# NVIDIA/makani

Measured on AMD Instinct MI355X. Metric: SFNO train samples/sec at 721x1440x73ch, higher is better.
Workload: dtype bf16; 1 GPU; sfno_sc3_layers8_edim384; grid=721x1440, channels=73, global_batch=1, parallelism=dp1, spectral_arithmetic=x3, multistep_count=1, multistep_checkpoint=False, launch=hipGraph replay of the captured step, channel_gemm=hip (csrc/conv1x1.hip)

## Files before the change

include/makani_amd.h:

```cpp
#ifndef MAKANI_AMD_H
#define MAKANI_AMD_H

#ifdef __cplusplus
extern "C" {
#endif

#define MK_F32 0
#define MK_BF16 1

#define MK_EINVAL -1
#define MK_EUNSUP -2

#define MK_TRI_NONE 0
#define MK_TRI_ROW_GE 1
#define MK_TRI_K_GE 2
#define MK_TRI_ROW_LE 3
#define MK_TRI_K_LE 4

typedef struct MkGemm {
    const float* A;
    const float* B;
    float* C;
    long long a_batch, a_row, a_k;
    long long b_batch, b_col, b_k;
// ... 75 lines not shown
int mk_bias_gelu_fwd(const void* x, const float* bias, void* y, int dtype, long long planes, int channels,
                     long long hw, void* stream);
int mk_bias_gelu_bwd(const void* x, const float* bias, const void* gy, void* gx, float* sums, float* ws, int dtype,
                     long long planes, int channels, long long hw, void* stream);

int mk_quad_lp_chunks(long long hw);
int mk_quad_lp_fwd(const void* a, int a_dtype, const void* b, int b_dtype, const float* wgt, const float* q,
                   float* sums, float* ws, long long planes, long long hw, int mode, float p, void* stream);
int mk_quad_lp_bwd(const void* a, int a_dtype, const void* b, int b_dtype, const float* wgt, const float* q,
                   const float* g, void* da, void* db, long long planes, long long hw, int mode, float p, void* stream);

long long mk_spec_lp_blocks(int L, int M);
int mk_spec_lp_fwd(const float* S, const float* wgt, float* partial, int L, int M, long long R, int tri_off, int m_off,
                   float p, float w0, float w1, void* stream);
int mk_spec_lp_bwd(const float* S, const float* wgt, const float* g, float* dS, int L, int M, long long R, int tri_off,
                   int m_off, float p, float w0, float w1, void* stream);

int mk_spec_sep_mul(const float* x, const float* w, float* y, int L, int M, int Mw, int B, int Cp, int tri_off, int conj_w,
                    void* stream);
int mk_spec_sep_wgrad(const float* x, const float* gy, float* gw, int L, int M, int Mw, int B, int Cp, int tri_off, void* stream);
int mk_spec_diag_apply(const float* x, const float* w_c64, float* y, int L, int M, int B, int Cin, int Cout, int x_ld, int y_ld,
                       int y_pad, int tri_off, int dgrad, void* stream);
int mk_spec_diag_wgrad(const float* x, const float* gy, float* gw_c64, int L, int M, int B, int Cin, int Cout, int x_ld, int y_ld,
                       int tri_off, void* stream);

int mk_conv1x1_nn(const void* A, const void* X, void* Y, void* Ypre, const float* bias, const void* R, const void* G,
                  int M, int K, int lda, int B, long long N, int act, void* stream);
long long mk_conv1x1_wgrad_workspace(int M, int K, int B, long long N);
int mk_conv1x1_wgrad(const void* G, const void* X, float* dW, float* part, int M, int K, int B, long long N,
                     int accumulate, void* stream);
int mk_conv1x1_wgrad_fuses_bias(int M, int K, int B, long long N);
int mk_conv1x1_wgrad_bias(const void* G, const void* X, float* dW, float* dbias, float* part, int M, int K, int B, long long N,
                          int accumulate, void* stream);

int mk_adamw_step(float* p, const float* g, float* m, float* v, long long n, const float* grad_scale, float lr,
                  float beta1, float beta2, float eps, float weight_decay, int step, const float* step_state, void* stream);
int mk_adamw_advance(float* state, float beta1, float beta2, void* stream);
typedef struct MkAdamTensor {
    float* p;
    const float* g;
    float* m;
    float* v;
    long long n;
    void* p_bf16;
    void* p_bf16_t;
    int cols;
    int ld, ld_t;
} MkAdamTensor;
int mk_adamw_multi(const MkAdamTensor* tensors, int count, const float* grad_scale, float lr, float beta1, float beta2,
                   float eps, float weight_decay, int step, const float* step_state, void* stream);
long long mk_grad_norm_workspace(const MkAdamTensor* tensors, int count);
int mk_grad_clip_coef(const MkAdamTensor* tensors, int count, float max_norm, float* partial, float* out, void* stream);
long long mk_grad_norm_workspace_pre(const MkAdamTensor* tensors, int count, const MkAdamTensor* pre, int npre);
int mk_grad_clip_coef_pre(const MkAdamTensor* tensors, int count, const MkAdamTensor* pre, int npre, float max_norm, float* partial,
                          float* out, void* stream);

int mk_chan_layernorm_chunks(int C, long long P);
int mk_chan_layernorm_fwd(const void* x, int x_dtype, void* y, int y_dtype, float* stats, const float* gamma, const float* beta,
                          int B, int C, long long P, float eps, void* stream);
int mk_chan_layernorm_bwd(const void* x, int x_dtype, const void* gy, int g_dtype, void* gx, const float* stats,
                          const float* gamma, int B, int C, long long P, void* stream);
int mk_chan_layernorm_wgrad(const void* x, int x_dtype, const void* gy, int g_dtype, const float* stats, float* partial, int B,
                            int C, long long P, void* stream);

int mk_crps_chunks(long long hw);
int mk_crps(const void* f, int f_dtype, const void* obs, int o_dtype, const float* q, const float* w, const float* gout,
// ... 41 lines not shown
```

makani_amd/_lib.py:

```python
import ctypes as C
import os

import torch

_HERE = os.path.dirname(os.path.abspath(__file__))
LIB_PATH = os.environ.get("MAKANI_AMD_LIB") or os.path.join(_HERE, "libmakani_amd.so")

MK_F32, MK_BF16 = 0, 1
TRI_NONE, TRI_ROW_GE, TRI_K_GE, TRI_ROW_LE, TRI_K_LE = 0, 1, 2, 3, 4

c_ll, c_int, c_f, c_vp = C.c_longlong, C.c_int, C.c_float, C.c_void_p


class MkAdamTensor(C.Structure):
    _fields_ = [("p", C.c_void_p), ("g", C.c_void_p), ("m", C.c_void_p), ("v", C.c_void_p), ("n", C.c_longlong),
                ("p_bf16", C.c_void_p), ("p_bf16_t", C.c_void_p), ("cols", C.c_int), ("ld", C.c_int), ("ld_t", C.c_int)]


class MkGemm(C.Structure):
    _fields_ = [
        ("A", c_vp), ("B", c_vp), ("C", c_vp),
        ("a_batch", c_ll), ("a_row", c_ll), ("a_k", c_ll),
        ("b_batch", c_ll), ("b_col", c_ll), ("b_k", c_ll),
        ("c_batch", c_ll), ("c_row", c_ll), ("c_col", c_ll),
# ... 27 lines not shown
                      c_f, c_f, c_f, c_vp], c_int),
    "mk_irfft_rows": ([c_vp, c_vp, c_int, c_vp, C.POINTER(c_int), c_int, c_int, c_int, c_int, c_int, c_int, c_int,
                       c_f, c_f, c_f, c_vp], c_int),
    "mk_fft_seg_supported": ([c_int], c_int),
    "mk_rfft_rows_seg": ([c_vp, c_int, c_vp, c_vp, c_int, c_int, c_int, c_int, c_f, c_f, c_f, C.POINTER(MkFftSeg), c_vp], c_int),
    "mk_irfft_rows_seg": ([c_vp, c_vp, c_int, c_vp, c_int, c_int, c_int, c_int, c_f, c_f, c_f, C.POINTER(MkFftSeg), c_vp], c_int),
    "mk_weight_to_wlayout": ([c_vp, c_vp, c_int, c_int, c_int, c_int, c_int, c_vp], c_int),
    "mk_wlayout_to_weight_grad": ([c_vp, c_vp, c_int, c_int, c_int, c_int, c_int, c_vp], c_int),
    "mk_slayout_to_complex": ([c_vp, c_vp, c_int, c_int, c_int, c_int, c_int, c_int, c_int, c_vp], c_int),
    "mk_complex_to_slayout": ([c_vp, c_vp, c_int, c_int, c_int, c_int, c_int, c_vp], c_int),
    "mk_spec_sep_mul": ([c_vp, c_vp, c_vp, c_int, c_int, c_int, c_int, c_int, c_int, c_int, c_vp], c_int),
    "mk_spec_sep_wgrad": ([c_vp, c_vp, c_vp, c_int, c_int, c_int, c_int, c_int, c_int, c_vp], c_int),
    "mk_spec_diag_apply": ([c_vp, c_vp, c_vp, c_int, c_int, c_int, c_int, c_int, c_int, c_int, c_int, c_int, c_int, c_vp], c_int),
    "mk_spec_diag_wgrad": ([c_vp, c_vp, c_vp, c_int, c_int, c_int, c_int, c_int, c_int, c_int, c_int, c_vp], c_int),
    "mk_pointwise_chunks": ([c_ll, c_int, c_ll], c_int),
    "mk_plane_sums": ([c_vp, c_int, c_vp, c_vp, c_ll, c_ll, c_vp], c_int),
    "mk_instnorm_stats": ([c_vp, c_int, c_vp, c_vp, c_ll, c_ll, c_f, c_vp, c_f, c_vp], c_int),
    "mk_instnorm_merge": ([c_vp, c_vp, c_vp, c_ll, c_int, c_f, c_vp], c_int),
    "mk_instnorm_apply": ([c_vp, c_vp, c_int, c_vp, c_vp, c_vp, c_ll, c_int, c_ll, c_int, c_vp], c_int),
    "mk_instnorm_fused_chunks": ([c_ll, c_int, c_ll, c_int], c_int),
    "mk_instnorm_fwd_fused": ([c_vp, c_vp, c_int, c_vp, c_vp, c_vp, c_vp, c_vp, c_vp, c_ll, c_int, c_ll, c_f, c_int, c_vp], c_int),
    "mk_instnorm_bwd_fused": ([c_vp, c_vp, c_vp, c_int, c_vp, c_vp, c_vp, c_vp, c_vp, c_vp, c_vp, c_ll, c_int, c_ll, c_int, c_vp], c_int),
    "mk_instnorm_bwd": ([c_vp, c_vp, c_vp, c_int, c_vp, c_vp, c_vp, c_vp, c_vp, c_f, c_vp, c_vp, c_ll, c_int, c_ll, c_ll, c_int, c_int, c_vp], c_int),
    "mk_chan_layernorm_chunks": ([c_int, c_ll], c_int),
    "mk_chan_layernorm_fwd": ([c_vp, c_int, c_vp, c_int, c_vp, c_vp, c_vp, c_int, c_int, c_ll, c_f, c_vp], c_int),
    "mk_chan_layernorm_bwd": ([c_vp, c_int, c_vp, c_int, c_vp, c_vp, c_vp, c_int, c_int, c_ll, c_vp], c_int),
    "mk_chan_layernorm_wgrad": ([c_vp, c_int, c_vp, c_int, c_vp, c_vp, c_int, c_int, c_ll, c_vp], c_int),
    "mk_bias_gelu_fwd": ([c_vp, c_vp, c_vp, c_int, c_ll, c_int, c_ll, c_vp], c_int),
    "mk_conv1x1_nn": ([c_vp, c_vp, c_vp, c_vp, c_vp, c_vp, c_vp, c_int, c_int, c_int, c_int, c_ll, c_int, c_vp], c_int),
    "mk_conv1x1_wgrad_workspace": ([c_int, c_int, c_int, c_ll], c_ll),
    "mk_conv1x1_wgrad": ([c_vp, c_vp, c_vp, c_vp, c_int, c_int, c_int, c_ll, c_int, c_vp], c_int),
    "mk_conv1x1_wgrad_fuses_bias": ([c_int, c_int, c_int, c_ll], c_int),
    "mk_conv1x1_wgrad_bias": ([c_vp, c_vp, c_vp, c_vp, c_vp, c_int, c_int, c_int, c_ll, c_int, c_vp], c_int),
    "mk_adamw_step": ([c_vp, c_vp, c_vp, c_vp, c_ll, c_vp, c_f, c_f, c_f, c_f, c_f, c_int, c_vp, c_vp], c_int),
    "mk_adamw_advance": ([c_vp, c_f, c_f, c_vp], c_int),
    "mk_bias_gelu_bwd": ([c_vp, c_vp, c_vp, c_vp, c_vp, c_vp, c_int, c_ll, c_int, c_ll, c_vp], c_int),
    "mk_adamw_multi": ([c_vp, c_int, c_vp, c_f, c_f, c_f, c_f, c_f, c_int, c_vp, c_vp], c_int),
    "mk_instnorm_fwd": ([c_vp, c_vp, c_int, c_vp, c_vp, c_vp, c_vp, c_vp, c_vp, c_f, c_ll, c_int, c_ll, c_f, c_int, c_vp], c_int),
    "mk_grad_norm_workspace": ([c_vp, c_int], c_ll),
    "mk_grad_clip_coef": ([c_vp, c_int, c_f, c_vp, c_vp, c_vp], c_int),
    "mk_grad_norm_workspace_pre": ([c_vp, c_int, c_vp, c_int], c_ll),
    "mk_grad_clip_coef_pre": ([c_vp, c_int, c_vp, c_int, c_f, c_vp, c_vp, c_vp], c_int),
    "mk_spec_lp_blocks": ([c_int, c_int], c_ll),
    "mk_spec_lp_fwd": ([c_vp, c_vp, c_vp, c_int, c_int, c_ll, c_int, c_int, c_f, c_f, c_f, c_vp], c_int),
    "mk_spec_lp_bwd": ([c_vp, c_vp, c_vp, c_vp, c_int, c_int, c_ll, c_int, c_int, c_f, c_f, c_f, c_vp], c_int),
    "mk_crps_chunks": ([c_ll], c_int),
    "mk_crps": ([c_vp, c_int, c_vp, c_int, c_vp, c_vp, c_vp, c_vp, c_vp, c_int, c_int, c_int, c_ll, c_int, c_f, c_f, c_int, c_vp, c_vp], c_int),
    "mk_crps_complex": ([c_vp, c_vp, c_vp, c_vp, c_vp, c_vp, c_vp, c_int, c_int, c_int, c_ll, c_f, c_int, c_vp], c_int),
    "mk_disco_fwd": ([c_vp, c_vp, c_int, c_vp, c_vp, c_vp, c_vp, c_vp, c_vp, c_int, c_int, c_int, c_int, c_int, c_int, c_int, c_vp], c_int),
    "mk_disco_bwd": ([c_vp, c_vp, c_int, c_vp, c_vp, c_vp, c_vp, c_vp, c_int, c_int, c_int, c_int, c_int, c_int, c_vp], c_int),
    "mk_disco_bwd_same": ([c_vp, c_vp, c_int, c_vp, c_vp, c_vp, c_vp, c_vp, c_vp, c_int, c_int, c_int, c_int, c_int, c_int, c_vp], c_int),
    "mk_disco_runs_shape": ([c_int, c_int, c_int, c_int, c_int, c_vp, c_vp], c_int),
    "mk_disco_fused_shape": ([c_int, c_int, c_int, c_int, c_vp, c_vp], c_int),
    "mk_disco_fwd_fused": ([c_vp, c_vp, c_int, c_vp, c_vp, c_vp, c_vp, c_vp, c_int, c_int, c_int, c_int, c_int, c_int, c_vp], c_int),
    "mk_disco_fwd_runs": ([c_vp, c_vp, c_int, c_vp, c_vp, c_vp, c_vp, c_vp, c_int, c_int, c_int, c_int, c_int, c_int, c_int, c_int, c_int, c_vp], c_int),
    "mk_disco_bwd_runs": ([c_vp, c_vp, c_int, c_vp, c_vp, c_vp, c_vp, c_vp, c_int, c_int, c_int, c_int, c_int, c_int, c_int, c_int, c_int, c_int, c_vp], c_int),
    "mk_group_mix_supported": ([c_int, c_int], c_int),
    "mk_group_mix_blocks": ([c_ll, c_int, c_int], c_int),
    "mk_group_mix": ([c_vp, c_vp, c_vp, c_int, c_int, c_int, c_int, c_int, c_ll, c_vp], c_int),
    "mk_group_mix_wgrad": ([c_vp, c_vp, c_vp, c_int, c_int, c_int, c_int, c_int, c_ll, c_vp], c_int),
    "mk_resample_fwd": ([c_vp, c_vp, c_int, c_vp, c_vp, c_vp, c_vp, c_vp, c_vp, c_int, c_int, c_int, c_int, c_int, c_vp], c_int),
    "mk_resample_bwd": ([c_vp, c_vp, c_int, c_vp, c_vp, c_vp, c_vp, c_vp, c_vp, c_vp, c_vp, c_vp, c_int, c_int, c_int, c_int, c_int, c_vp], c_int),
    "mk_quad_lp_chunks": ([c_ll], c_int),
    "mk_quad_lp_fwd": ([c_vp, c_int, c_vp, c_int, c_vp, c_vp, c_vp, c_vp, c_ll, c_ll, c_int, c_f, c_vp], c_int),
    "mk_quad_lp_bwd": ([c_vp, c_int, c_vp, c_int, c_vp, c_vp, c_vp, c_vp, c_vp, c_ll, c_ll, c_int, c_f, c_vp], c_int),
}
# ... 74 lines not shown
```

makani_amd/csrc/conv1x1.hip:

```cpp
#include <stdlib.h>
#include <type_traits>

#include "common.h"

#ifndef MK_ASTAT_EPI_DRAIN
#define MK_ASTAT_EPI_DRAIN 0
#endif
#ifndef MK_A2_PRIO
#define MK_A2_PRIO 1
#endif
#ifndef MK_ASTAT_DIAG
#define MK_ASTAT_DIAG 0
#endif
#if MK_ASTAT_DIAG
__device__ unsigned long long g_astat_diag[16];
#define MK_AS_STAMP(k)                                              \
    do {                                                            \
        const unsigned long long t_ = __builtin_readcyclecounter(); \
        dg[k] += t_ - tprev;                                        \
        tprev = t_;                                                 \
    } while (0)
#else
#define MK_AS_STAMP(k)
#endif
// ... 1335 lines not shown
                store_tiles(ra[0], rb[0], 0);
                __syncthreads();
            }
        }
    }

    float* out = p.part + (long long)sp * p.M * p.K;
#pragma unroll
    for (int i = 0; i < 2; ++i)
#pragma unroll
        for (int j = 0; j < 2; ++j) {
            const int c = c0 + wn * 64 + j * 32 + l31;
#pragma unroll
            for (int r = 0; r < 16; ++r) {
                const int m = m0 + wm * 64 + i * 32 + (r & 3) + 8 * (r >> 2) + 4 * lh;
                if (m < p.M && c < p.K) out[(long long)m * p.K + c] = acc[i][j][r];
            }
        }
}

struct ConvWgR {
    const u16* P;
    const u16* Q;
    float* part;
    int RP, RQ, B, S, slabs, qslabs;
    int ldo;
    long long N;
    long long chunk;
    float* bias_part;
};


template <int WP, int WQ, int WTP, int WTQ, bool SWAP>
__global__ __launch_bounds__(512, 2) void conv_wgrad_ring_kernel(const ConvWgR p) {
#if defined(__HIP_DEVICE_COMPILE__)
    static_assert(WP * WQ == 8, "8 waves");
    constexpr int TP = WP * WTP * 32, TQ = WQ * WTQ * 32;
    constexpr int BK = 64;
    constexpr int STAGE = (TP + TQ) * 128;
    constexpr int NI = (TP + TQ) / 64;
    constexpr int NIP = TP / 64;
    static_assert(TP % 64 == 0 && TQ == 384, "row groups; Q is fetched by 2 x 3 DMA pieces per wave");
    __shared__ __attribute__((aligned(1024))) unsigned char smem[2 * STAGE];

    const int bid = xcd_remap(blockIdx.x, gridDim.x);
    const int slab = bid % p.slabs;
    const int qs = (bid / p.slabs) % p.qslabs;
    const int q0 = qs * TQ;
    const int sp = bid / (p.slabs * p.qslabs);
    const int splits_per_b = p.S / p.B;
    const int b = sp / splits_per_b;
    const long long nbeg = (long long)(sp % splits_per_b) * p.chunk;
    const long long nend = min(p.N, nbeg + p.chunk);
    const int nk = nbeg < nend ? (int)((nend - nbeg + BK - 1) / BK) : 0;

    const int tid = threadIdx.x, lane = tid & 63, wave = tid >> 6;
    const int wp = wave / WQ, wq = wave % WQ;
    const int l31 = lane & 31, lh = lane >> 5;

    const int c_log = (lane & 7) ^ ((((wave & 1) << 2) + (lane >> 4)) & 7);
    const unsigned rowbytes = (unsigned)(p.N * 2);
    unsigned voff[NI];
#pragma unroll
    for (int i = 0; i < NI; ++i) {
        const int rg = wave + 8 * i;
        int row;
        if (i < NIP) row = min(rg * 8 + (lane >> 3), p.RP - 1 - slab * TP);
        else row = min((rg - TP / 8) * 8 + (lane >> 3), p.RQ - 1 - q0);
        voff[i] = (unsigned)row * rowbytes + (unsigned)c_log * 16u;
    }
    const v4i_t rsP = make_rsrc(p.P + ((long long)b * p.RP + slab * TP) * p.N);
    const v4i_t rsQ = make_rsrc(p.Q + ((long long)b * p.RQ + q0) * p.N);
    const unsigned lds_w = lds_addr(smem) + __builtin_amdgcn_readfirstlane(wave) * 1024;

    auto issue = [&](int kt, int stage) {
        const long long n = nbeg + (long long)kt * BK;
        const unsigned soff = (unsigned)__builtin_amdgcn_readfirstlane((int)(unsigned)(n * 2));
        const unsigned dst = lds_w + stage * STAGE;
// ... 71 lines not shown
        asm volatile("s_waitcnt lgkmcnt(0)" ::: "memory");
        __builtin_amdgcn_s_barrier();
        if (kt + 2 < nk) issue(kt + 2, kt & 1);
    }

    if (bias_wave) {
        const int RG = SWAP ? p.RQ : p.RP;
#pragma unroll
        for (int i = 0; i < WTG; ++i) {
            const float tot = rsum[i] + __shfl_xor(rsum[i], 32);
            const int m = SWAP ? q0 + (wq * WTQ + i) * 32 + l31 : slab * TP + (wp * WTP + i) * 32 + l31;
            if (lh == 0 && m < RG) p.bias_part[((long long)sp * NSH + bshare) * RG + m] = tot;
        }
    }

    float* out = p.part + (long long)sp * ((long long)(SWAP ? p.RQ : p.RP) * p.ldo);
#pragma unroll
    for (int i = 0; i < WTP; ++i)
#pragma unroll
        for (int j = 0; j < WTQ; ++j) {
            const int prow0 = slab * TP + (wp * WTP + i) * 32, qrow0 = q0 + (wq * WTQ + j) * 32;
#pragma unroll
            for (int r = 0; r < 16; ++r) {
                const int rr = (r & 3) + 8 * (r >> 2) + 4 * lh;
                const int m = SWAP ? qrow0 + rr : prow0 + rr;
                const int k = SWAP ? prow0 + l31 : qrow0 + l31;
                const bool ok = SWAP ? (m < p.RQ && k < p.RP) : (m < p.RP && k < p.RQ);
                if (ok) out[(long long)m * p.ldo + k] = acc[i][j][r];
            }
        }
#endif
}

__global__ void reduce_splits(const float* __restrict__ part, float* __restrict__ out, long long n, int S, int accumulate) {
    const long long i = (long long)blockIdx.x * blockDim.x + threadIdx.x;
    if (i >= n) return;
    float s = accumulate ? out[i] : 0.f;
    int k = 0;
    for (; k + 8 <= S; k += 8) {
        float v[8];
#pragma unroll
        for (int u = 0; u < 8; ++u) v[u] = part[(long long)(k + u) * n + i];
#pragma unroll
        for (int u = 0; u < 8; ++u) s += v[u];
    }
    for (; k < S; ++k) s += part[(long long)k * n + i];
    out[i] = s;
}

__global__ void reduce_splits4(const float4* __restrict__ part, float4* __restrict__ out, long long n4, int S, int accumulate) {
    const long long i = (long long)blockIdx.x * blockDim.x + threadIdx.x;
    if (i >= n4) return;
    float4 s = accumulate ? out[i] : make_float4(0.f, 0.f, 0.f, 0.f);
    int k = 0;
    for (; k + 8 <= S; k += 8) {
        float4 v[8];
#pragma unroll
        for (int u = 0; u < 8; ++u) v[u] = part[(long long)(k + u) * n4 + i];
#pragma unroll
        for (int u = 0; u < 8; ++u) s.x += v[u].x, s.y += v[u].y, s.z += v[u].z, s.w += v[u].w;
    }
    for (; k < S; ++k) {
        const float4 v = part[(long long)k * n4 + i];
        s.x += v.x, s.y += v.y, s.z += v.z, s.w += v.w;
    }
    out[i] = s;
}

}

#if MK_ASTAT_DIAG
extern "C" int mk_astat_diag_read(unsigned long long* out, int reset) {
    if (hipMemcpyFromSymbol(out, HIP_SYMBOL(g_astat_diag), sizeof(unsigned long long) * 16) != hipSuccess) return 1;
    if (reset) {
        unsigned long long z[16] = {};
        if (hipMemcpyToSymbol(HIP_SYMBOL(g_astat_diag), z, sizeof(z)) != hipSuccess) return 1;
    }
    return 0;
}
#endif

extern "C" int mk_conv1x1_nn(const void* A, const void* X, void* Y, void* Ypre, const float* bias, const void* R,
                             const void* G, int M, int K, int lda, int B, long long N, int act, void* stream) {
    MK_REQUIRE(A && X && Y, "conv1x1_nn: null pointer");
    MK_REQUIRE(M > 0 && K > 0 && B > 0 && N > 0, "conv1x1_nn: bad shape M=%d K=%d B=%d N=%lld", M, K, B, N);
    MK_REQUIRE((lda % 8) == 0 && lda >= K, "conv1x1_nn: lda=%d must be a multiple of 8 and >= K=%d", lda, K);
    MK_REQUIRE((N % 8) == 0, "conv1x1_nn: pixel count %lld must be a multiple of 8", N);
    MK_REQUIRE((((uintptr_t)A | (uintptr_t)X) & 15) == 0, "conv1x1_nn: operands must be 16-byte aligned");
    static const int nt_env = [] { const char* e = getenv("MAKANI_AMD_CONV_NT"); return e ? atoi(e) : -1; }();
    const long long out_bytes = (long long)B * M * N * 2;
    const int nt = nt_env >= 0 ? (nt_env == 1 || (nt_env == 2 && out_bytes * ((act && Ypre) ? 2 : 1) <= (256ll << 20))) : (out_bytes <= (256ll << 20));
    ConvNN p{(const u16*)A, (const u16*)X, (u16*)Y, (u16*)Ypre, bias, (const u16*)R, (const u16*)G, M, K, lda, B, N, act, nt};
    static const bool force_tile = [] { const char* e = getenv("MAKANI_AMD_CONV_NN"); return e && e[0] == 't'; }();
    static const bool no_astat = [] { const char* e = getenv("MAKANI_AMD_CONV_NN"); return e && e[0] == 'r'; }();
    if (!force_tile && !no_astat && lda == 80 && K > 64 && K <= 80 && M >= 256 && (long long)M * N * 2 < (1ll << 31) &&
        (long long)K * N * 2 < (1ll << 32) && N >= 64 && !(R && G) && !((R || G) && act && Ypre)) {
        const bool epi_loads = R || G;
        const int slabs = (M + 383) / 384;
        const long long tn = (N + 63) / 64;
// ... 132 lines not shown
    if (per_b > maxs) per_b = maxs;
    long long chunk = (N + per_b - 1) / per_b;
    chunk = (chunk + 127) / 128 * 128;
    pl.chunk = chunk;
    pl.S = per_b * B;
    return pl;
}
}

extern "C" long long mk_conv1x1_wgrad_workspace(int M, int K, int B, long long N) {
    const WgPlan pl = wgrad_plan(M, K, B, N);
    return pl.S * (long long)M * K + pl.S * (long long)M;
}

extern "C" int mk_conv1x1_wgrad_fuses_bias(int M, int K, int B, long long N) {
    return wgrad_plan(M, K, B, N).ring ? 1 : 0;
}

static int conv1x1_wgrad_impl(const void* G, const void* X, float* dW, float* dbias, float* part, int M, int K, int B, long long N,
                              int accumulate, void* stream);

extern "C" int mk_conv1x1_wgrad(const void* G, const void* X, float* dW, float* part, int M, int K, int B, long long N,
                                int accumulate, void* stream) {
    return conv1x1_wgrad_impl(G, X, dW, nullptr, part, M, K, B, N, accumulate, stream);
}

extern "C" int mk_conv1x1_wgrad_bias(const void* G, const void* X, float* dW, float* dbias, float* part, int M, int K, int B,
                                     long long N, int accumulate, void* stream) {
    MK_REQUIRE(dbias, "conv1x1_wgrad_bias: null pointer");
    MK_REQUIRE(wgrad_plan(M, K, B, N).ring, "conv1x1_wgrad_bias: this shape runs the tile kernel, which does not form the bias gradient");
    return conv1x1_wgrad_impl(G, X, dW, dbias, part, M, K, B, N, accumulate, stream);
}

static int conv1x1_wgrad_impl(const void* G, const void* X, float* dW, float* dbias, float* part, int M, int K, int B, long long N,
                              int accumulate, void* stream) {
    MK_REQUIRE(G && X && dW && part, "conv1x1_wgrad: null pointer");
    MK_REQUIRE(M > 0 && K > 0 && B > 0 && N > 0 && (N % 8) == 0, "conv1x1_wgrad: bad shape");
    const WgPlan pl = wgrad_plan(M, K, B, N);
    hipStream_t s = (hipStream_t)stream;
    if (pl.ring) {
        ConvWgR p{};
        p.P = (const u16*)(pl.swap ? X : G);
        p.Q = (const u16*)(pl.swap ? G : X);
        p.RP = pl.swap ? K : M;
        p.RQ = pl.swap ? M : K;
        p.part = part, p.B = B, p.S = (int)pl.S, p.slabs = pl.slabs, p.qslabs = pl.qslabs, p.ldo = K, p.N = N, p.chunk = pl.chunk;
        p.bias_part = dbias ? part + pl.S * (long long)M * K : nullptr;
        const dim3 grid((unsigned)(pl.slabs * pl.qslabs * pl.S)), blk(512);
        if (pl.tp == 256) {
            if (pl.swap) hipLaunchKernelGGL((conv_wgrad_ring_kernel<2, 4, 4, 3, true>), grid, blk, 0, s, p);
            else hipLaunchKernelGGL((conv_wgrad_ring_kernel<2, 4, 4, 3, false>), grid, blk, 0, s, p);
        } else {
            if (pl.swap) hipLaunchKernelGGL((conv_wgrad_ring_kernel<2, 4, 3, 3, true>), grid, blk, 0, s, p);
            else hipLaunchKernelGGL((conv_wgrad_ring_kernel<2, 4, 3, 3, false>), grid, blk, 0, s, p);
        }
    } else {
        const int tm = (M + 127) / 128, tk = (K + 127) / 128;
        ConvWg p{(const u16*)G, (const u16*)X, part, M, K, B, (int)pl.S, N, pl.chunk};
        hipLaunchKernelGGL(conv_wgrad_kernel<128>, dim3((unsigned)(tm * tk * pl.S)), dim3(NT), 0, s, p, tm, tk);
    }
    const long long n = (long long)M * K;
    if (n % 4 == 0 && (((uintptr_t)part | (uintptr_t)dW) & 15) == 0)
        hipLaunchKernelGGL(reduce_splits4, dim3((unsigned)((n / 4 + 255) / 256)), dim3(256), 0, s, (const float4*)part, (float4*)dW,
                           n / 4, (int)pl.S, accumulate);
    else
        hipLaunchKernelGGL(reduce_splits, dim3((unsigned)((n + 255) / 256)), dim3(256), 0, s, part, dW, n, (int)pl.S, accumulate);
    if (dbias)
        hipLaunchKernelGGL(reduce_splits, dim3((unsigned)((M + 255) / 256)), dim3(256), 0, s, part + pl.S * n, dbias, (long long)M,
                           (int)pl.S, 0);
    return mk_check_launch("mk_conv1x1_wgrad");
}
```

makani_amd/ops.py:

```python
import ctypes as C
import os
import weakref
from dataclasses import dataclass

import numpy as np
import torch

from . import _lib
from ._lib import MkGemm, check, dtype_code, lib, ptr, stream
from . import legendre as _leg


def round4(n: int) -> int:
    return (n + 3) // 4 * 4


GEMM_MODE = os.environ.get("MAKANI_AMD_GEMM", "auto")
if GEMM_MODE not in ("auto", "x6", "x3", "fp32"):
    raise ValueError(f"MAKANI_AMD_GEMM={GEMM_MODE!r}: expected auto, x6, x3 or fp32")


def gemm_mode() -> str:
    if GEMM_MODE != "auto":
        return GEMM_MODE
# ... 872 lines not shown
    N = H * W
    y = torch.empty((B, M, H, W), dtype=torch.bfloat16, device=x.device)
    ypre = torch.empty_like(y) if (act and want_pre) else None
    bf = bias.float().contiguous() if bias is not None else None
    r = residual.contiguous() if residual is not None else None
    g = gelu_grad_of.contiguous() if gelu_grad_of is not None else None
    extra = (ypre is not None) + (r is not None) + (g is not None)
    with _timed(f"conv1x1_nn_m{M}_k{K}_n{N}", flops=2.0 * B * M * K * N, nbytes=2.0 * B * N * (M * (1 + extra) + K)):
        check(lib().mk_conv1x1_nn(ptr(A), ptr(x), ptr(y), ptr(ypre), ptr(bf), ptr(r), ptr(g), M, K, lda, B, N,
                                  1 if act else 0, stream()), "mk_conv1x1_nn")
    return y, ypre


def conv1x1_wgrad(g: torch.Tensor, x: torch.Tensor, want_bias: bool = False):
    B, M, H, W = g.shape
    K = x.shape[1]
    N = H * W
    g, x = g.contiguous(), x.contiguous()
    nws = lib().mk_conv1x1_wgrad_workspace(M, K, B, N)
    part = torch.empty((nws,), dtype=torch.float32, device=g.device)
    dW = torch.empty((M, K), dtype=torch.float32, device=g.device)
    fused = want_bias and bool(lib().mk_conv1x1_wgrad_fuses_bias(M, K, B, N))
    with _timed(f"conv1x1_wgrad_m{M}_k{K}_n{N}", flops=2.0 * B * M * K * N, nbytes=2.0 * B * N * (M + K)):
        if fused:
            db = torch.empty((M,), dtype=torch.float32, device=g.device)
            check(lib().mk_conv1x1_wgrad_bias(ptr(g), ptr(x), ptr(dW), ptr(db), ptr(part), M, K, B, N, 0, stream()), "mk_conv1x1_wgrad_bias")
        else:
            check(lib().mk_conv1x1_wgrad(ptr(g), ptr(x), ptr(dW), ptr(part), M, K, B, N, 0, stream()), "mk_conv1x1_wgrad")
    if not want_bias:
        return dW
    return dW, (db if fused else _sum_planes(g))


def _sum_planes(t: torch.Tensor) -> torch.Tensor:
    if not (t.is_cuda and t.dim() == 4 and t.dtype in (torch.bfloat16, torch.float32)):
        raise RuntimeError("makani_amd ops need 4-d bf16 / fp32 GPU tensors (the HIP path has no CPU fallback)")
    t = t.contiguous()
    B, Cc, H, W = t.shape
    sums = torch.empty((2, B * Cc), dtype=torch.float32, device=t.device)
    check(lib().mk_plane_sums(ptr(t), dtype_code(t), ptr(sums), ptr(_ws(B * Cc, H * W, t.dtype, t.device)), B * Cc, H * W,
                              stream()), "mk_plane_sums")
    return _batch_sum(sums, B, Cc)[0]


class Conv1x1Fn(torch.autograd.Function):

    @staticmethod
    def forward(ctx, x, weight, bias, residual):
        M, K = weight.shape[0], weight.shape[1]
        A, At = weight_operands(weight, need_t=ctx.needs_input_grad[0])
        y, _ = conv1x1_nn(A, K, x, bias=bias, residual=residual)
        ctx.save_for_backward(x, weight, At)
        ctx.has_bias = bias is not None
        ctx.has_res = residual is not None
        return y

    @staticmethod
    def backward(ctx, gy):
        x, weight, At = ctx.saved_tensors
        M, K = weight.shape[0], weight.shape[1]
        gy = gy.contiguous()
        gx = gw = gb = gr = None
        if ctx.needs_input_grad[0]:
            gx, _ = conv1x1_nn(At, M, gy)
        want_b = ctx.has_bias and ctx.needs_input_grad[2]
        if ctx.needs_input_grad[1]:
# ... 2 lines not shown
                gw = gw.view_as(weight)
            else:
                gw = conv1x1_wgrad(gy, x).view_as(weight)
        elif want_b:
            gb = _sum_planes(gy)
        if ctx.has_res and ctx.needs_input_grad[3]:
            gr = gy
        return gx, gw, gb, gr


class ConvGeluConvFn(torch.autograd.Function):

    @staticmethod
    def forward(ctx, x, w1, b1, w2, b2):
        H1, K = w1.shape[0], w1.shape[1]
        M = w2.shape[0]
        A1, A1t = weight_operands(w1, need_t=ctx.needs_input_grad[0])
        A2, A2t = weight_operands(w2, need_t=True)
        h, a1 = conv1x1_nn(A1, K, x, bias=b1, act=True, want_pre=True)
        y, _ = conv1x1_nn(A2, H1, h, bias=b2)
        ctx.save_for_backward(x, w1, w2, a1, h, A1t, A2t)
        ctx.has_b = (b1 is not None, b2 is not None)
        return y

    @staticmethod
    def backward(ctx, gy):
        x, w1, w2, a1, h, A1t, A2t = ctx.saved_tensors
        H1, K = w1.shape[0], w1.shape[1]
        M = w2.shape[0]
        gy = gy.contiguous()
        ga1, _ = conv1x1_nn(A2t, M, gy, gelu_grad_of=a1)
        gw2 = gb2 = gw1 = gb1 = None
        want_b2, want_b1 = ctx.has_b[1] and ctx.needs_input_grad[4], ctx.has_b[0] and ctx.needs_input_grad[2]
        if ctx.needs_input_grad[3] and want_b2:
            gw2, gb2 = conv1x1_wgrad(gy, h, want_bias=True)
            gw2 = gw2.view_as(w2)
        else:
            gw2 = conv1x1_wgrad(gy, h).view_as(w2) if ctx.needs_input_grad[3] else None
            gb2 = _sum_planes(gy) if want_b2 else None
        if ctx.needs_input_grad[1] and want_b1:
            gw1, gb1 = conv1x1_wgrad(ga1, x, want_bias=True)
            gw1 = gw1.view_as(w1)
        else:
            gw1 = conv1x1_wgrad(ga1, x).view_as(w1) if ctx.needs_input_grad[1] else None
            gb1 = _sum_planes(ga1) if want_b1 else None
        gx = None
        if ctx.needs_input_grad[0]:
            gx, _ = conv1x1_nn(A1t, H1, ga1)
        return gx, gw1, gb1, gw2, gb2


def want_bf16_shadow(param):
    param._mk_want_bf16 = True


def _shadow_valid(weight):
    return (getattr(weight, "_mk_shadow", None) is not None and getattr(weight, "_mk_shadow_version", -1) == weight._version
            and getattr(weight, "_mk_shadow_ptr", 0) == weight.data_ptr() and weight._mk_shadow.device == weight.device)


def cast_weight(weight, dtype):
    if dtype == weight.dtype:
        return weight
    if dtype == torch.bfloat16 and _shadow_valid(weight):
        K = weight.numel() // weight.shape[0]
        sh = weight._mk_shadow
# ... 247 lines not shown
```

Measured before the change: 28.13 samples/s.

## Group the two MLP weight-gradient GEMMs and share one split-K reduction

Adds a grouped weight-gradient path for the MLP backward that plans both conv1x1 wgrad problems together. Each ring kernel can still launch separately, or with a 'fill' setting run as one combined launch that balances split-K counts to fill the device. The split reductions for both weight and bias gradients are merged into a single reduce kernel. The aim is fewer launches and better occupancy of the small wgrad GEMMs, at the cost of a larger shared workspace and more planning complexity.

```diff
diff --git a/include/makani_amd.h b/include/makani_amd.h
--- a/include/makani_amd.h
+++ b/include/makani_amd.h
@@ -131,6 +131,15 @@
 int mk_conv1x1_wgrad_fuses_bias(int M, int K, int B, long long N);
 int mk_conv1x1_wgrad_bias(const void* G, const void* X, float* dW, float* dbias, float* part, int M, int K, int B, long long N,
                           int accumulate, void* stream);
+
+#define MK_WGRAD_GROUP_MAX 4
+#define MK_WGRAD_GROUP_PLAN_FIELDS 10
+int mk_conv1x1_wgrad_group_enabled(void);
+long long mk_conv1x1_wgrad_group_workspace(int n, const int* M, const int* K, const int* B, const long long* N);
+int mk_conv1x1_wgrad_group_plan(int n, const int* M, const int* K, const int* B, const long long* N, long long* out);
+int mk_conv1x1_wgrad_group(int n, const void* const* G, const void* const* X, float* const* dW, float* const* dbias,
+                           const int* M, const int* K, const int* B, const long long* N, const int* accumulate, float* part,
+                           void* stream);
 
 int mk_adamw_step(float* p, const float* g, float* m, float* v, long long n, const float* grad_scale, float lr,
                   float beta1, float beta2, float eps, float weight_decay, int step, const float* step_state, void* stream);
diff --git a/makani_amd/_lib.py b/makani_amd/_lib.py
--- a/makani_amd/_lib.py
+++ b/makani_amd/_lib.py
@@ -83,6 +83,10 @@
     "mk_conv1x1_wgrad": ([c_vp, c_vp, c_vp, c_vp, c_int, c_int, c_int, c_ll, c_int, c_vp], c_int),
     "mk_conv1x1_wgrad_fuses_bias": ([c_int, c_int, c_int, c_ll], c_int),
     "mk_conv1x1_wgrad_bias": ([c_vp, c_vp, c_vp, c_vp, c_vp, c_int, c_int, c_int, c_ll, c_int, c_vp], c_int),
+    "mk_conv1x1_wgrad_group_enabled": ([], c_int),
+    "mk_conv1x1_wgrad_group_workspace": ([c_int, c_vp, c_vp, c_vp, c_vp], c_ll),
+    "mk_conv1x1_wgrad_group_plan": ([c_int, c_vp, c_vp, c_vp, c_vp, c_vp], c_int),
+    "mk_conv1x1_wgrad_group": ([c_int, c_vp, c_vp, c_vp, c_vp, c_vp, c_vp, c_vp, c_vp, c_vp, c_vp, c_vp], c_int),
     "mk_adamw_step": ([c_vp, c_vp, c_vp, c_vp, c_ll, c_vp, c_f, c_f, c_f, c_f, c_f, c_int, c_vp, c_vp], c_int),
     "mk_adamw_advance": ([c_vp, c_f, c_f, c_vp], c_int),
     "mk_bias_gelu_bwd": ([c_vp, c_vp, c_vp, c_vp, c_vp, c_vp, c_int, c_ll, c_int, c_ll, c_vp], c_int),
diff --git a/makani_amd/csrc/conv1x1.hip b/makani_amd/csrc/conv1x1.hip
--- a/makani_amd/csrc/conv1x1.hip
+++ b/makani_amd/csrc/conv1x1.hip
@@ -1391,7 +1391,7 @@
 
 
 template <int WP, int WQ, int WTP, int WTQ, bool SWAP>
-__global__ __launch_bounds__(512, 2) void conv_wgrad_ring_kernel(const ConvWgR p) {
+__device__ __forceinline__ void conv_wgrad_ring_body(const ConvWgR& p, const int bid, unsigned char* smem) {
 #if defined(__HIP_DEVICE_COMPILE__)
     static_assert(WP * WQ == 8, "8 waves");
     constexpr int TP = WP * WTP * 32, TQ = WQ * WTQ * 32;
@@ -1400,9 +1400,7 @@
     constexpr int NI = (TP + TQ) / 64;
     constexpr int NIP = TP / 64;
     static_assert(TP % 64 == 0 && TQ == 384, "row groups; Q is fetched by 2 x 3 DMA pieces per wave");
-    __shared__ __attribute__((aligned(1024))) unsigned char smem[2 * STAGE];
-
-    const int bid = xcd_remap(blockIdx.x, gridDim.x);
+
     const int slab = bid % p.slabs;
     const int qs = (bid / p.slabs) % p.qslabs;
     const int q0 = qs * TQ;
@@ -1540,8 +1538,43 @@
 #endif
 }
 
-__global__ void reduce_splits(const float* __restrict__ part, float* __restrict__ out, long long n, int S, int accumulate) {
-    const long long i = (long long)blockIdx.x * blockDim.x + threadIdx.x;
+template <int WP, int WQ, int WTP, int WTQ, bool SWAP>
+__global__ __launch_bounds__(512, 2) void conv_wgrad_ring_kernel(const ConvWgR p) {
+#if defined(__HIP_DEVICE_COMPILE__)
+    __shared__ __attribute__((aligned(1024))) unsigned char smem[2 * (WP * WTP + WQ * WTQ) * 32 * 128];
+    conv_wgrad_ring_body<WP, WQ, WTP, WTQ, SWAP>(p, xcd_remap(blockIdx.x, gridDim.x), smem);
+#endif
+}
+
+constexpr int WG_GROUP_MAX = MK_WGRAD_GROUP_MAX;
+struct ConvWgG {
+    ConvWgR p[WG_GROUP_MAX];
+    int first[WG_GROUP_MAX + 1];
+    int kind[WG_GROUP_MAX];
+    int n;
+};
+
+__global__ __launch_bounds__(512, 2) void conv_wgrad_ring_group_kernel(const ConvWgG g) {
+#if defined(__HIP_DEVICE_COMPILE__)
+    __shared__ __attribute__((aligned(1024))) unsigned char smem[2 * (256 + 384) * 128];
+    const int bid = xcd_remap(blockIdx.x, gridDim.x);
+    int i = 0;
+#pragma unroll
+    for (int j = 1; j < WG_GROUP_MAX; ++j)
+        if (j < g.n && bid >= g.first[j]) i = j;
+    i = __builtin_amdgcn_readfirstlane(i);
+    const int local = bid - g.first[i];
+    switch (g.kind[i]) {
+        case 0: conv_wgrad_ring_body<2, 4, 4, 3, false>(g.p[i], local, smem); break;
+        case 1: conv_wgrad_ring_body<2, 4, 4, 3, true>(g.p[i], local, smem); break;
+        case 2: conv_wgrad_ring_body<2, 4, 3, 3, false>(g.p[i], local, smem); break;
+        default: conv_wgrad_ring_body<2, 4, 3, 3, true>(g.p[i], local, smem); break;
+    }
+#endif
+}
+
+__device__ __forceinline__ void reduce_splits_at(const float* __restrict__ part, float* __restrict__ out, long long n, int S,
+                                                 int accumulate, long long i) {
     if (i >= n) return;
     float s = accumulate ? out[i] : 0.f;
     int k = 0;
@@ -1556,8 +1589,12 @@
     out[i] = s;
 }
 
-__global__ void reduce_splits4(const float4* __restrict__ part, float4* __restrict__ out, long long n4, int S, int accumulate) {
-    const long long i = (long long)blockIdx.x * blockDim.x + threadIdx.x;
+__global__ void reduce_splits(const float* __restrict__ part, float* __restrict__ out, long long n, int S, int accumulate) {
+    reduce_splits_at(part, out, n, S, accumulate, (long long)blockIdx.x * blockDim.x + threadIdx.x);
+}
+
+__device__ __forceinline__ void reduce_splits4_at(const float4* __restrict__ part, float4* __restrict__ out, long long n4, int S,
+                                                  int accumulate, long long i) {
     if (i >= n4) return;
     float4 s = accumulate ? out[i] : make_float4(0.f, 0.f, 0.f, 0.f);
     int k = 0;
@@ -1573,6 +1610,33 @@
         s.x += v.x, s.y += v.y, s.z += v.z, s.w += v.w;
     }
     out[i] = s;
+}
+
+__global__ void reduce_splits4(const float4* __restrict__ part, float4* __restrict__ out, long long n4, int S, int accumulate) {
+    reduce_splits4_at(part, out, n4, S, accumulate, (long long)blockIdx.x * blockDim.x + threadIdx.x);
+}
+
+struct RedSeg {
+    const float* part;
+    float* out;
+    long long n;
+    int S, accumulate, vec;
+    int first;
+};
+struct RedGroup {
+    RedSeg s[2 * WG_GROUP_MAX];
+    int n;
+};
+
+__global__ __launch_bounds__(256) void reduce_splits_group(const RedGroup g) {
+    int i = 0;
+#pragma unroll
+    for (int j = 1; j < 2 * WG_GROUP_MAX; ++j)
+        if (j < g.n && (int)blockIdx.x >= g.s[j].first) i = j;
+    const RedSeg& r = g.s[i];
+    const long long e = (long long)((int)blockIdx.x - r.first) * 256 + threadIdx.x;
+    if (r.vec) reduce_splits4_at((const float4*)r.part, (float4*)r.out, r.n, r.S, r.accumulate, e);
+    else reduce_splits_at(r.part, r.out, r.n, r.S, r.accumulate, e);
 }
 
 }
@@ -1771,6 +1835,25 @@
     return conv1x1_wgrad_impl(G, X, dW, dbias, part, M, K, B, N, accumulate, stream);
 }
 
+static void launch_wgrad_ring(const WgPlan& pl, const void* G, const void* X, float* part, float* bias_part, int M, int K, int B,
+                              long long N, hipStream_t s) {
+    ConvWgR p{};
+    p.P = (const u16*)(pl.swap ? X : G);
+    p.Q = (const u16*)(pl.swap ? G : X);
+    p.RP = pl.swap ? K : M;
+    p.RQ = pl.swap ? M : K;
+    p.part = part, p.B = B, p.S = (int)pl.S, p.slabs = pl.slabs, p.qslabs = pl.qslabs, p.ldo = K, p.N = N, p.chunk = pl.chunk;
+    p.bias_part = bias_part;
+    const dim3 grid((unsigned)(pl.slabs * pl.qslabs * pl.S)), blk(512);
+    if (pl.tp == 256) {
+        if (pl.swap) hipLaunchKernelGGL((conv_wgrad_ring_kernel<2, 4, 4, 3, true>), grid, blk, 0, s, p);
+        else hipLaunchKernelGGL((conv_wgrad_ring_kernel<2, 4, 4, 3, false>), grid, blk, 0, s, p);
+    } else {
+        if (pl.swap) hipLaunchKernelGGL((conv_wgrad_ring_kernel<2, 4, 3, 3, true>), grid, blk, 0, s, p);
+        else hipLaunchKernelGGL((conv_wgrad_ring_kernel<2, 4, 3, 3, false>), grid, blk, 0, s, p);
+    }
+}
+
 static int conv1x1_wgrad_impl(const void* G, const void* X, float* dW, float* dbias, float* part, int M, int K, int B, long long N,
                               int accumulate, void* stream) {
     MK_REQUIRE(G && X && dW && part, "conv1x1_wgrad: null pointer");
@@ -1778,21 +1861,7 @@
     const WgPlan pl = wgrad_plan(M, K, B, N);
     hipStream_t s = (hipStream_t)stream;
     if (pl.ring) {
-        ConvWgR p{};
-        p.P = (const u16*)(pl.swap ? X : G);
-        p.Q = (const u16*)(pl.swap ? G : X);
-        p.RP = pl.swap ? K : M;
-        p.RQ = pl.swap ? M : K;
-        p.part = part, p.B = B, p.S = (int)pl.S, p.slabs = pl.slabs, p.qslabs = pl.qslabs, p.ldo = K, p.N = N, p.chunk = pl.chunk;
-        p.bias_part = dbias ? part + pl.S * (long long)M * K : nullptr;
-        const dim3 grid((unsigned)(pl.slabs * pl.qslabs * pl.S)), blk(512);
-        if (pl.tp == 256) {
-            if (pl.swap) hipLaunchKernelGGL((conv_wgrad_ring_kernel<2, 4, 4, 3, true>), grid, blk, 0, s, p);
-            else hipLaunchKernelGGL((conv_wgrad_ring_kernel<2, 4, 4, 3, false>), grid, blk, 0, s, p);
-        } else {
-            if (pl.swap) hipLaunchKernelGGL((conv_wgrad_ring_kernel<2, 4, 3, 3, true>), grid, blk, 0, s, p);
-            else hipLaunchKernelGGL((conv_wgrad_ring_kernel<2, 4, 3, 3, false>), grid, blk, 0, s, p);
-        }
+        launch_wgrad_ring(pl, G, X, part, dbias ? part + pl.S * (long long)M * K : nullptr, M, K, B, N, s);
     } else {
         const int tm = (M + 127) / 128, tk = (K + 127) / 128;
         ConvWg p{(const u16*)G, (const u16*)X, part, M, K, B, (int)pl.S, N, pl.chunk};
@@ -1809,3 +1878,189 @@
                            (int)pl.S, 0);
     return mk_check_launch("mk_conv1x1_wgrad");
 }
+
+namespace {
+int wgrad_group_choice() {
+    static int v = -1;
+    if (v < 0) {
+        const char* e = getenv("MAKANI_AMD_WGRAD_GROUP");
+        v = !e ? 1 : (e[0] == '0' ? 0 : (e[0] == 'f' ? 2 : 1));
+    }
+    return v;
+}
+
+struct WgGroupPlan {
+    WgPlan pl[WG_GROUP_MAX];
+    bool grouped[WG_GROUP_MAX];
+    int first[WG_GROUP_MAX + 1];
+    long long part_off[WG_GROUP_MAX];
+    long long bias_off[WG_GROUP_MAX];
+    long long ws;
+    int ngrouped;
+};
+
+long long round_up4(long long v) { return (v + 3) / 4 * 4; }
+
+void wgrad_group_fill(WgGroupPlan& g, int n, const int* B, const long long* N, const long long* tiles, long long* per_b) {
+    long long maxs[WG_GROUP_MAX] = {};
+    double total = 0;
+    for (int i = 0; i < n; ++i) {
+        if (!g.grouped[i]) continue;
+        maxs[i] = (N[i] + 511) / 512;
+        total += (double)tiles[i] * N[i] * g.pl[i].tp;
+    }
+    const double target = total / 256.0;
+    auto set_splits = [&](int i, long long s) {
+        if (s > maxs[i]) s = maxs[i];
+        if (s < 1) s = 1;
+        const long long chunk = ((N[i] + s - 1) / s + 63) / 64 * 64;
+        g.pl[i].chunk = chunk;
+        per_b[i] = (N[i] + chunk - 1) / chunk;
+    };
+    long long wgs = 0;
+    for (int i = 0; i < n; ++i) {
+        if (!g.grouped[i]) continue;
+        set_splits(i, (long long)((double)N[i] * g.pl[i].tp / target));
+        wgs += tiles[i] * per_b[i];
+    }
+    for (;;) {
+        int best = -1;
+        double bw = 0;
+        for (int i = 0; i < n; ++i) {
+            if (!g.grouped[i] || per_b[i] >= maxs[i] || wgs + tiles[i] > 256) continue;
+            const double w = (double)g.pl[i].chunk * g.pl[i].tp;
+            if (w > bw) bw = w, best = i;
+        }
+        if (best < 0) break;
+        const long long before = per_b[best];
+        long long want = before + 1;
+        do set_splits(best, want++); while (per_b[best] == before && want <= maxs[best]);
+        if (per_b[best] == before || wgs + tiles[best] * (per_b[best] - before) > 256) {
+            set_splits(best, before);
+            maxs[best] = per_b[best];
+            continue;
+        }
+        wgs += tiles[best] * (per_b[best] - before);
+    }
+}
+
+WgGroupPlan wgrad_group_plan(int n, const int* M, const int* K, const int* B, const long long* N) {
+    WgGroupPlan g{};
+    for (int i = 0; i < n; ++i) {
+        g.pl[i] = wgrad_plan(M[i], K[i], B[i], N[i]);
+        g.grouped[i] = wgrad_group_choice() != 0 && g.pl[i].ring;
+        g.ngrouped += g.grouped[i] ? 1 : 0;
+    }
+    if (g.ngrouped < 2) {
+        for (int i = 0; i < n; ++i) g.grouped[i] = false;
+        g.ngrouped = 0;
+    }
+    long long tiles[WG_GROUP_MAX] = {}, per_b[WG_GROUP_MAX] = {};
+    for (int i = 0; i < n; ++i) {
+        if (!g.grouped[i]) continue;
+        tiles[i] = (long long)g.pl[i].slabs * g.pl[i].qslabs * B[i];
+        per_b[i] = g.pl[i].S / B[i];
+    }
+    if (wgrad_group_choice() == 2) wgrad_group_fill(g, n, B, N, tiles, per_b);
+    int first = 0;
+    long long off = 0;
+    for (int i = 0; i < n; ++i) {
+        g.first[i] = first;
+        g.part_off[i] = off;
+        const long long mk = (long long)M[i] * K[i];
+        if (g.grouped[i]) {
+            g.pl[i].S = per_b[i] * B[i];
+            first += (int)(tiles[i] * per_b[i]);
+            g.bias_off[i] = off + round_up4(g.pl[i].S * mk);
+            off = g.bias_off[i] + round_up4(g.pl[i].S * M[i]);
+        } else {
+            g.bias_off[i] = off + g.pl[i].S * mk;
+            off += round_up4(g.pl[i].S * mk + g.pl[i].S * M[i]);
+        }
+    }
+    g.first[n] = first;
+    g.ws = off;
+    return g;
+}
+
+bool group_args_ok(int n, const int* M, const int* K, const int* B, const long long* N) {
+    if (n < 1 || n > WG_GROUP_MAX || !M || !K || !B || !N) return false;
+    for (int i = 0; i < n; ++i)
+        if (M[i] <= 0 || K[i] <= 0 || B[i] <= 0 || N[i] <= 0 || (N[i] % 8) != 0) return false;
+    return true;
+}
+}
+
+extern "C" int mk_conv1x1_wgrad_group_enabled(void) { return wgrad_group_choice() != 0 ? 1 : 0; }
+
+extern "C" long long mk_conv1x1_wgrad_group_workspace(int n, const int* M, const int* K, const int* B, const long long* N) {
+    if (!group_args_ok(n, M, K, B, N)) return -1;
+    return wgrad_group_plan(n, M, K, B, N).ws;
+}
+
+extern "C" int mk_conv1x1_wgrad_group_plan(int n, const int* M, const int* K, const int* B, const long long* N, long long* out) {
+    if (!group_args_ok(n, M, K, B, N) || !out) return -1;
+    const WgGroupPlan g = wgrad_group_plan(n, M, K, B, N);
+    for (int i = 0; i < n; ++i) {
+        long long* o = out + (long long)i * MK_WGRAD_GROUP_PLAN_FIELDS;
+        o[0] = g.grouped[i] ? 1 : 0, o[1] = g.pl[i].tp, o[2] = g.pl[i].slabs, o[3] = g.pl[i].qslabs, o[4] = g.pl[i].S;
+        o[5] = g.pl[i].chunk, o[6] = g.first[i], o[7] = g.part_off[i], o[8] = g.bias_off[i], o[9] = g.pl[i].swap ? 1 : 0;
+    }
+    return g.first[n];
+}
+
+extern "C" int mk_conv1x1_wgrad_group(int n, const void* const* G, const void* const* X, float* const* dW, float* const* dbias,
+                                      const int* M, const int* K, const int* B, const long long* N, const int* accumulate,
+                                      float* part, void* stream) {
+    MK_REQUIRE(group_args_ok(n, M, K, B, N), "conv1x1_wgrad_group: bad shape or more than MK_WGRAD_GROUP_MAX problems");
+    MK_REQUIRE(G && X && dW && part, "conv1x1_wgrad_group: null pointer");
+    MK_REQUIRE((((uintptr_t)part) & 15) == 0, "conv1x1_wgrad_group: workspace must be 16-byte aligned");
+    const WgGroupPlan g = wgrad_group_plan(n, M, K, B, N);
+    hipStream_t s = (hipStream_t)stream;
+    const bool one_ring_launch = wgrad_group_choice() == 2;
+    ConvWgG kg{};
+    RedGroup rg{};
+    int rblocks = 0;
+    for (int i = 0; i < n; ++i) {
+        MK_REQUIRE(G[i] && X[i] && dW[i], "conv1x1_wgrad_group: null pointer");
+        float* db = dbias ? dbias[i] : nullptr;
+        const int acc = accumulate ? accumulate[i] : 0;
+        const WgPlan& pl = g.pl[i];
+        if (!g.grouped[i]) {
+            MK_REQUIRE(!db || pl.ring, "conv1x1_wgrad_group: this member runs the tile kernel, which does not form the bias gradient");
+            const int rc = conv1x1_wgrad_impl(G[i], X[i], dW[i], db, part + g.part_off[i], M[i], K[i], B[i], N[i], acc, stream);
+            if (rc != 0) return rc;
+            continue;
+        }
+        if (!one_ring_launch)
+            launch_wgrad_ring(pl, G[i], X[i], part + g.part_off[i], db ? part + g.bias_off[i] : nullptr, M[i], K[i], B[i], N[i], s);
+        ConvWgR& p = kg.p[kg.n];
+        p.P = (const u16*)(pl.swap ? X[i] : G[i]);
+        p.Q = (const u16*)(pl.swap ? G[i] : X[i]);
+        p.RP = pl.swap ? K[i] : M[i];
+        p.RQ = pl.swap ? M[i] : K[i];
+        p.part = part + g.part_off[i], p.B = B[i], p.S = (int)pl.S, p.slabs = pl.slabs, p.qslabs = pl.qslabs, p.ldo = K[i];
+        p.N = N[i], p.chunk = pl.chunk;
+        p.bias_part = db ? part + g.bias_off[i] : nullptr;
+        kg.first[kg.n] = g.first[i];
+        kg.kind[kg.n] = (pl.swap ? 1 : 0) | (pl.tp == 192 ? 2 : 0);
+        ++kg.n;
+        const long long mk = (long long)M[i] * K[i];
+        RedSeg& r = rg.s[rg.n++];
+        const bool vec = mk % 4 == 0 && (((uintptr_t)dW[i]) & 15) == 0;
+        r.part = p.part, r.out = dW[i], r.n = vec ? mk / 4 : mk, r.S = (int)pl.S, r.accumulate = acc, r.vec = vec ? 1 : 0;
+        r.first = rblocks;
+        rblocks += (int)((r.n + 255) / 256);
+        if (db) {
+            RedSeg& rb = rg.s[rg.n++];
+            rb.part = p.bias_part, rb.out = db, rb.n = M[i], rb.S = (int)pl.S, rb.accumulate = 0, rb.vec = 0, rb.first = rblocks;
+            rblocks += (M[i] + 255) / 256;
+        }
+    }
+    if (kg.n > 0) {
+        kg.first[kg.n] = g.first[n];
+        if (one_ring_launch) hipLaunchKernelGGL(conv_wgrad_ring_group_kernel, dim3((unsigned)g.first[n]), dim3(512), 0, s, kg);
+        hipLaunchKernelGGL(reduce_splits_group, dim3((unsigned)rblocks), dim3(256), 0, s, rg);
+    }
+    return mk_check_launch("mk_conv1x1_wgrad_group");
+}
diff --git a/makani_amd/ops.py b/makani_amd/ops.py
--- a/makani_amd/ops.py
+++ b/makani_amd/ops.py
@@ -928,6 +928,63 @@
     return dW, (db if fused else _sum_planes(g))
 
 
+def wgrad_group_enabled() -> bool:
+    return bool(lib().mk_conv1x1_wgrad_group_enabled())
+
+
+WGRAD_GROUP_MAX = 4
+
+
+def conv1x1_wgrad_group(problems, accumulate_into=None):
+    if not 1 <= len(problems) <= WGRAD_GROUP_MAX:
+        raise ValueError(f"a group holds 1 ... {WGRAD_GROUP_MAX} weight gradients")
+    acc = list(accumulate_into) if accumulate_into is not None else [None] * len(problems)
+    out = [None] * len(problems)
+    members = []
+    for i, (g, x, want_bias) in enumerate(problems):
+        B, M, H, W = g.shape
+        K, N = x.shape[1], H * W
+        if wgrad_group_enabled() and lib().mk_conv1x1_wgrad_fuses_bias(M, K, B, N):
+            members.append((i, g.contiguous(), x.contiguous(), bool(want_bias), M, K, B, N))
+            continue
+        r = conv1x1_wgrad(g, x, want_bias=want_bias)
+        dW, db = r if want_bias else (r, None)
+        if acc[i] is not None:
+            dW = acc[i].add_(dW)
+        out[i] = (dW, db)
+    if len(members) == 1:
+        i, g, x, want_bias = members[0][:4]
+        r = conv1x1_wgrad(g, x, want_bias=want_bias)
+        dW, db = r if want_bias else (r, None)
+        out[i] = (acc[i].add_(dW) if acc[i] is not None else dW, db)
+        members = []
+    if members:
+        n = len(members)
+        dev = members[0][1].device
+        arr_i, arr_l, arr_p = C.c_int * n, C.c_longlong * n, C.c_void_p * n
+        Ms, Ks, Bs = arr_i(*[m[4] for m in members]), arr_i(*[m[5] for m in members]), arr_i(*[m[6] for m in members])
+        Ns = arr_l(*[m[7] for m in members])
+        nws = lib().mk_conv1x1_wgrad_group_workspace(n, Ms, Ks, Bs, Ns)
+        if nws < 0:
+            raise RuntimeError("mk_conv1x1_wgrad_group_workspace: bad group")
+        part = torch.empty((nws,), dtype=torch.float32, device=dev)
+        dWs = [acc[m[0]] if acc[m[0]] is not None else torch.empty((m[4], m[5]), dtype=torch.float32, device=dev) for m in members]
+        dbs = [torch.empty((m[4],), dtype=torch.float32, device=dev) if m[3] else None for m in members]
+        for m, dW in zip(members, dWs):
+            if dW.shape != (m[4], m[5]) or dW.dtype != torch.float32 or not dW.is_contiguous():
+                raise ValueError("accumulate_into: contiguous fp32 (M, K) tensors")
+        flops = sum(2.0 * m[6] * m[4] * m[5] * m[7] for m in members)
+        nbytes = sum(2.0 * m[6] * m[7] * (m[4] + m[5]) for m in members)
+        with _timed(f"conv1x1_wgrad_group{n}", flops=flops, nbytes=nbytes):
+            check(lib().mk_conv1x1_wgrad_group(n, arr_p(*[ptr(m[1]) for m in members]), arr_p(*[ptr(m[2]) for m in members]),
+                                               arr_p(*[ptr(t) for t in dWs]), arr_p(*[ptr(t) for t in dbs]), Ms, Ks, Bs, Ns,
+                                               arr_i(*[int(acc[m[0]] is not None) for m in members]), ptr(part), stream()),
+                  "mk_conv1x1_wgrad_group")
+        for m, dW, db in zip(members, dWs, dbs):
+            out[m[0]] = (dW, db)
+    return out
+
+
 def _sum_planes(t: torch.Tensor) -> torch.Tensor:
     if not (t.is_cuda and t.dim() == 4 and t.dtype in (torch.bfloat16, torch.float32)):
         raise RuntimeError("makani_amd ops need 4-d bf16 / fp32 GPU tensors (the HIP path has no CPU fallback)")
@@ -996,6 +1053,13 @@
         ga1, _ = conv1x1_nn(A2t, M, gy, gelu_grad_of=a1)
         gw2 = gb2 = gw1 = gb1 = None
         want_b2, want_b1 = ctx.has_b[1] and ctx.needs_input_grad[4], ctx.has_b[0] and ctx.needs_input_grad[2]
+        if ctx.needs_input_grad[3] and ctx.needs_input_grad[1] and wgrad_group_enabled():
+            (gw2, gb2), (gw1, gb1) = conv1x1_wgrad_group([(gy, h, want_b2), (ga1, x, want_b1)])
+            gw2, gw1 = gw2.view_as(w2), gw1.view_as(w1)
+            gx = None
+            if ctx.needs_input_grad[0]:
+                gx, _ = conv1x1_nn(A1t, H1, ga1)
+            return gx, gw1, gb1, gw2, gb2
         if ctx.needs_input_grad[3] and want_b2:
             gw2, gb2 = conv1x1_wgrad(gy, h, want_bias=True)
             gw2 = gw2.view_as(w2)
```

Result: no change. 28.11 samples/s, median of 4 (-0.1%).
